# Project-SEA-Stack/HydroChrono

Measured on AMD Instinct MI355X. Metric: hydro-force evals/sec (all bodies), higher is better.
Workload: dtype f64

## Files before the change

hydrochrono_amd/csrc/hc_context.hpp:

```cpp
#pragma once
#include <hip/hip_runtime.h>

#include <chrono>
#include <cmath>
#include <deque>
#include <stdexcept>
#include <string>
#include <vector>

#include "../../include/hydrochrono_amd.h"
#include "hc_direct.hpp"
#include "hc_kernels.hpp"
#include "hc_plan.hpp"

namespace hc {

struct Error : std::runtime_error {
    int status;
    Error(int st, const std::string& what) : std::runtime_error(what), status(st) {}
};

#define HC_HIP(expr)                                                                                          \
    do {                                                                                                      \
        hipError_t _e = (expr);                                                                               \
// ... 126 lines not shown
    std::vector<std::vector<double>> tris;
    int items = 0, chunks = 0;
    std::vector<int> runs;
    DeviceBuffer<double> panel, tri, state, part, out;
    DeviceBuffer<int> chunk, off;
    PinnedBuffer<double> h_state, h_out;
    bool pts_dirty = true;
    DeviceBuffer<double> pt;
    DeviceBuffer<int> pbody;
    DeviceBuffer<int> pidx, tidx;
};

struct BodyHost {
    bool have_props = false, have_lin = false, have_ainf = false, have_rirf = false, have_rao = false, have_exirf = false;
    double disp_vol = 0.0, cg[3] = {0, 0, 0}, cb[3] = {0, 0, 0};
    double lin[36]  = {0};
    std::vector<double> ainf;
    std::vector<double> rao_w;
    std::vector<double> rao_mag;
    std::vector<double> rao_phase;
    std::vector<double> hd_dir;
    std::vector<double> hd_w;
    std::vector<double> hd_mag;
    std::vector<double> hd_phase;
    std::vector<double> exirf_t;
    std::vector<double> exirf_f;
};

struct StepTail {
    bool pending = false, rad = false, waves = false, block = false, direct = false, caller_waits = false;
    int m = 0, H = 0;
    hipStream_t stream = nullptr;
};

struct AheadPass {
    bool active = false;
    unsigned long long plan_serial = 0;
    int slices = 0, issued = 0;
    int per_slice = 0;
    bool reduced = false;
    bool concurrent = false;
    bool has_exc = false;
    int Hcap = 0;
    int head0 = 0, Hv = 0;
    double t_first = 0.0, t_last = 0.0;
    double rad_once = 0.0, exc_once = 0.0;
    BlockArgs args;
};

struct ExGroup {
    int first_body = 0, off = 0, L = 0;
    double tau_front = 0.0, tau_back = 0.0;
};

enum WaveKind { kWaveNone = 0, kWaveRegular = 1, kWaveIrregular = 2, kWaveSpectral = 3 };

enum EventKind { kEvConvPlain = 0, kEvPass = 1, kEvStep = 2, kEvScatter = 3, kEvConvExc = 4, kEvMiniPass = 5, kEvTail = 6 };
struct EventPair {
    hipEvent_t a = nullptr, b = nullptr;
    int kind = 0;
    double waves_share = 0.0;
};

}

struct hc_ctx {
    int N = 0, b0 = 0, b1 = 0, nloc = 0, D = 0, Dloc = 0, device = 0;
    hipStream_t stream = nullptr;
    hipStream_t stream_am = nullptr;
    hipEvent_t ev_fin = nullptr, ev_bg = nullptr;
    bool bg_pending = false;
    hipStream_t last_stream = nullptr;
    bool have_last_stream   = false;
    hc::DirectQueue* dq = nullptr;
    bool direct_ready   = false;
    std::string direct_why;
    std::string direct_how = "direct AQL dispatch";
    int path            = 0;
    hc::DirectKernel dk_finalize_slot;
    hc::DirectKernel dk_step_hot[2];
    bool step_hot = false;
    int step_halves = 1;
    bool slot_state = false;
    hc::DirectKernel dk_finalize, dk_scatter, dk_reduce, dk_block16, dk_block32, dk_block64, dk_mini16, dk_mini32, dk_narrow, dk_wide, dk_added_mass, dk_step, dk_near;
    hc::StepTail tail;
    int pending_step  = 0;
    double pending_t  = 0.0;
    int pending_am    = 0;
    bool lost         = false;
    int arm_mode = 1;
    bool arm_after_step = false, arm_after_am = false;
    std::chrono::steady_clock::time_point t_step_end{}, t_am_end{};
    bool have_t_step_end = false, have_t_am_end = false;
    int busy_caller_steps   = 0;
    std::string err;

    bool have_sim = false;
    double rho = 0, g = 0, depth = 0;
    double gsys[3] = {0.0, 0.0, -9.81};
    std::vector<hc::BodyHost> bodies;

    int S = 0;
    std::vector<double> tau, width;
    hc::DeviceBuffer<double> dK, dKproc, d_tau, d_width, d_stage;
    int ntiles = 0, Dpad = 0, ngp = 0, mt = 1, ngroups = 0;
    int conv_mode = 0;
    bool proc_ready = false;
    hc_tapered_direct_options taper{};
    std::string diagnostics_dir;
    bool finalized = false;

    std::deque<double> times;
    std::deque<double> retired;
    int head = -1, Hcap = 0, HcapT = 0;
    hc::DeviceBuffer<double> d_ring_t, d_ring_v, d_ring_vT;
    long long rewinds = 0;
    bool have_prev = false, have_prev_device = false;
    double prev_time = -1.0, prev_time_device = -1.0;

    hc::DeviceBuffer<double> d_lin, d_cg, d_cbmcg, d_vol, d_ainf, d_vec_w, d_vec_R;
    std::vector<double> ainf_host;

    int wave_kind = hc::kWaveNone;
    int wave_nb_arg = 0;
    double reg_amp = 0, reg_omega = 0, reg_wavenumber = 0;
    std::vector<double> reg_mag, reg_phase;
    hc::DeviceBuffer<double> d_reg_mag;
    hc_irregular_wave_params irr{};
    int eta_mode = 0;
    int L = 0, Lpad = 0, nf = 0, nt = 0;
    std::vector<double> ex_tau, ex_width, ex_vals;
    std::vector<hc::ExGroup> ex_groups;
    std::vector<int> ex_group_of;
    std::vector<double> spec_f, spec_S, spec_df, spec_phase, spec_k;
    std::vector<double> eta_t, eta;
    bool eta_record = false;
    std::vector<double> rec_t, rec_eta;
    double eta_h = 0.0;
    std::vector<int> rec_m;
    std::vector<double> rec_amp;
    double rec_mean = 0.0, rec_share = 0.0, rec_rms = 0.0;
    bool record_components() const { return wave_kind == hc::kWaveIrregular && eta_record && !rec_amp.empty(); }
    void drop_record_components() {
        rec_m.clear();
        rec_amp.clear();
        rec_mean = rec_share = rec_rms = 0.0;
    }
    hc::DeviceBuffer<double> d_kex, d_ex_tau, d_ex_width, d_eta_t, d_eta;
    hc::DeviceBuffer<double> d_spec_mag, d_spec_phase, d_spec_amp, d_spec_omega, d_spec_phi;
    unsigned long long wave_serial = 0;
    std::vector<double> wave_dir;

    hc::KinTableCopy kin;
    hc::DeviceBuffer<double> d_kin_io;

    hc::SideLane mor, nl;
    hc::Order2Part mor2, nl2;
    hc::MorisonData morison;
    hc::SurfaceData surface;

    hc::QtfTerm drift, sum;

    hipStream_t stream_wk2 = nullptr;
    hc::Wk2TableSet wk2;
    hc::DeviceBuffer<double> d_wk2_io;

    int chunk_gp = 0, nchunks_rad = 0, chunk_gp_ex = 0, nchunks_ex = 0, ngp_ex = 0;
// ... 98 lines not shown
```

hydrochrono_amd/csrc/hc_internal.hpp:

```cpp
#pragma once
#include <dlfcn.h>
#include <fcntl.h>
#include <unistd.h>
#include <xmmintrin.h>

#include <algorithm>
#include <chrono>
#include <cmath>
#include <cstdint>
#include <cstdio>
#include <cstdlib>
#include <cstring>
#include <fstream>
#include <limits>
#include <memory>
#include <string>
#include <vector>

#include "hc_context.hpp"
#include "hc_history.hpp"
#include "hc_host_math.hpp"

namespace hc {
void eta_synthesis_fft(const std::vector<double>& t, const std::vector<double>& amp, const std::vector<double>& omega,
// ... 61 lines not shown
#define HC_TUNE_INT(name, fallback) ::hc::detail::env_int(name, fallback)
#else
#define HC_TUNE_INT(name, fallback) (fallback)
#endif
void setup_panel_geometry(hc_ctx* c);
hc::Panel rad_panel(const hc_ctx* c);
void choose_conv_config(hc_ctx* c);
void choose_exc_config(hc_ctx* c);
void alloc_partials(hc_ctx* c);
int far_chunk_gp(const hc_ctx* c);
int far_chunks_per_slice(const hc_ctx* c);
int default_pass_slices(const hc_ctx* c);
int default_pass_ahead(const hc_ctx* c);
bool pass_ahead_size_ok(const hc_ctx* c);
bool pass_ahead_possible(const hc_ctx* c);
void reset_schedule_state(hc_ctx* c);
void ensure_processed(hc_ctx* c);
void check_device_flag(hc_ctx* c);
void stage_state(hc_ctx* c, const double* pos, const double* rpy, const double* linvel, const double* angvel);
std::string library_dir();
bool direct_selftest_rewrites(hc_ctx* c, hc::DirectQueue* q, int lane, bool* abandon);
void setup_direct(hc_ctx* c);

struct ExcitationGrid {
    std::vector<hc::ExGroup> groups;
    std::vector<int> group_of;
    std::vector<double> tau, width, vals;
    int L = 0;
    double tau_min = 0.0, tau_max = 0.0;
};
ExcitationGrid resample_excitation(hc_ctx* c, double dt);
void upload_excitation(hc_ctx* c, const ExcitationGrid& ex);
void commit_excitation(hc_ctx* c, ExcitationGrid& ex);
void drop_lookahead_excitation(hc_ctx* c);

struct RaoBracket {
    int k0, k1;
    double fr;
};
inline RaoBracket rao_bracket_clamped(double omega, double w_back, int nw) {
    const double dw = w_back / static_cast<double>(nw);
    double idx = omega / dw - 1;
    idx        = std::min(std::max(idx, 0.0), static_cast<double>(nw - 1));
    const int k0 = std::min(static_cast<int>(std::floor(idx)), nw - 2 >= 0 ? nw - 2 : 0);
    const int k1 = std::min(k0 + 1, nw - 1);
    return RaoBracket{k0, k1, idx - k0};
}
inline RaoBracket rao_bracket_regular(double omega, double w_back, int nw) {
    const double dw      = w_back / static_cast<double>(nw);
    const double idx_des = (omega / dw) - 1;
    const int k0         = static_cast<int>(std::floor(idx_des));
    return RaoBracket{k0, k0 + 1, idx_des - std::floor(idx_des)};
}
inline void rao_bracket_check(const RaoBracket& br, int nw) {
    if (br.k0 < 0 || br.k0 + 1 >= nw) throw Error(HC_ERR_OUT_OF_RANGE, "regular wave frequency outside the BEM frequency list");
}
void apply_wave_directions(hc_ctx* c, const std::vector<double>& theta, bool commit, bool force);

struct StepFlags {
    bool hs = true, rad = true, waves = true;
    bool scratch_out = false;
};
struct HostState {
    const double *pos, *rpy, *linvel, *angvel;
    double canary;
};
void enqueue_step(hc_ctx* c, double t, const double* d_state, double* d_user_out, hipStream_t stream, StepFlags f,
                  unsigned long long* host_tagged = nullptr, unsigned long long seq = 0, bool defer_tail = false, const HostState* host_state = nullptr);
void enqueue_tail(hc_ctx* c);

bool wave_window_ok(const hc_ctx* c, double t);
int live_samples(const hc_ctx* c, double t_query);
double* rows_P(hc_ctx* c, bool next);
double* rows_E(hc_ctx* c, bool next);

struct StepViews {
    hc::Panel kex;
    hc::EtaTable ex;
};
StepViews make_views(const hc_ctx* c);
struct PassSetup {
    hc::BlockArgs b;
    bool exc_block = false;
    double rad_once = 0.0, exc_once = 0.0, bytes_steps = 0.0;
};
PassSetup make_pass(hc_ctx* c, bool with_exc, bool next_block, int head_lags = 0);
void issue_pass_chunks(hc_ctx* c, const PassSetup& ps, int first, int last, bool with_items, hipStream_t stream, bool direct, int lane = 0);
struct TailRows {
    const double* tail[hc::kTailLevelsMax] = {nullptr, nullptr, nullptr};
    int j0[hc::kTailLevelsMax]             = {0, 0, 0};
};
void issue_pass_reduce(hc_ctx* c, const PassSetup& ps, double* P, double* E, hipStream_t stream, bool direct, int lane = 0, const TailRows* tail = nullptr);
void launch_pass(hc_ctx* c, hipStream_t stream, bool with_exc, bool direct = false, bool spec_goes_on = false);
void spec_drop(hc_ctx* c, bool k_changed);
void spec_build_khat(hc_ctx* c, hc_ctx::SpectralLevel& lev);
void launch_mini_pass(hc_ctx* c, int i0, hipStream_t stream, bool direct, int next_kw = 0, int lane = 0);
void ahead_drop(hc_ctx* c);
void ahead_issue_slice(hc_ctx* c, hipStream_t stream, bool direct);
void ahead_begin(hc_ctx* c, hipStream_t stream, bool with_exc, bool direct);
bool ahead_expected(const hc_ctx* c, unsigned long long ended_serial);
bool ahead_adoptable(const hc_ctx* c, unsigned long long ended_serial);
bool pass_lane_ready(hc_ctx* c);
void pass_lane_drain(hc_ctx* c);

}
}
```

hydrochrono_amd/csrc/hc_kernels.hip:

```cpp
#include "hc_kernels.hpp"

#include <algorithm>
#include <cstdint>
#include <cstdlib>

namespace hc {

static constexpr int kConvThreads = 256;
static constexpr int kWave        = 64;

typedef double dvec2 __attribute__((ext_vector_type(2)));
typedef double dvec2u __attribute__((ext_vector_type(2), aligned(8)));
typedef double dvec4 __attribute__((ext_vector_type(4)));

__host__ __device__ inline size_t panel_offset(int ngp, int row, int f) {
    const int rt = row >> 4, ri = row & 15, gp = f >> 3, j = (f >> 2) & 1, kk = f & 3;
    return ((static_cast<size_t>(rt) * ngp + gp) * 64 + (kk * 16 + ri)) * 2 + j;
}

__global__ void __launch_bounds__(256) relayout_rirf_kernel(const double* __restrict__ Kb, double* __restrict__ K, int ngp, int D, int S,
                                                             int row0, double scale) {
    const size_t F   = (size_t)S * D;
    const size_t gid = (size_t)blockIdx.x * blockDim.x + threadIdx.x;
    if (gid >= 6 * F) return;
// ... 768 lines not shown
        else block_rad_stream<MT, (NB > 1) ? 2 : R, NB, false>(a, chunk, grp, front, t_wo, t_wn, t_oo, t_on);
    }
    const int RG      = a.ngroups;
    const int n_items = a.nchunks_ex * NB * RG;
    if (n_items > 0) {
        __shared__ int s_item;
        for (;;) {
            __syncthreads();
            if (threadIdx.x == 0) s_item = atomicAdd(a.item_counter, 1);
            __syncthreads();
            const int it = s_item;
            if (it >= n_items) break;
            const int e = it / (NB * RG), rem = it - e * (NB * RG), tb = rem / RG, rg = rem - tb * RG;
            block_exc_work<MT>(a, rg, e, 16 * tb, front);
        }
    }
}

template <class KernelT>
static void allow_dynamic_lds(KernelT kernel, size_t smem, size_t& granted) {
    if (smem > 64 * 1024 && smem > granted) {
        (void)hipFuncSetAttribute(reinterpret_cast<const void*>(kernel), hipFuncAttributeMaxDynamicSharedMemorySize, (int)smem);
        granted = smem;
    }
}

template <int MT, int R>
static void launch_conv_block_mt(const BlockArgs& b, int nblocks, size_t smem, hipStream_t stream) {
    static size_t granted16 = 0, granted32 = 0;
    if (b.depth == 32) {
        allow_dynamic_lds(conv_block_kernel<MT, R + 1, 2>, smem, granted32);
        hipLaunchKernelGGL((conv_block_kernel<MT, R + 1, 2>), dim3(nblocks), dim3(kConvThreads), smem, stream, b);
    } else {
        allow_dynamic_lds(conv_block_kernel<MT, R, 1>, smem, granted16);
        hipLaunchKernelGGL((conv_block_kernel<MT, R, 1>), dim3(nblocks), dim3(kConvThreads), smem, stream, b);
    }
}

#ifdef HC_TUNING
static void launch_conv_block64(const BlockArgs& b, int nblocks, size_t smem, hipStream_t stream) {
    static size_t granted = 0;
    allow_dynamic_lds(conv_block_kernel<kBlock64MT, 4, 4, 1>, smem, granted);
    hipLaunchKernelGGL((conv_block_kernel<kBlock64MT, 4, 4, 1>), dim3(nblocks), dim3(kConvThreads), smem, stream, b);
}
#endif

BlockLaunch block_launch_config(const BlockArgs& a, int mt, BlockArgs* b) {
    BlockLaunch l;
    const int nlaunch = (a.chunk_last > 0 ? a.chunk_last : a.nchunks) - a.chunk_first;
    l.nblocks = ((nlaunch + 7) >> 3) * 8 * a.ngroups;
    *b        = a;
    b->lds_front_doubles = max(4 * kUWave, 4 * mt * 256);
    l.smem    = (size_t)b->lds_front_doubles * sizeof(double) + (size_t)max(1, a.max_steps_per_chunk) * b->depth * 24;
#ifdef HC_TUNING
    if (a.depth == 64) {
        l.MT  = kBlock64MT;
        l.NB  = 4;
        l.R   = 4;
        l.WPS = 1;
        return l;
    }
#endif
    l.MT  = (mt == 6 || mt == 4 || mt == 2) ? mt : 1;
    const int R16 = l.MT == 6 ? 3 : 4;
    l.NB  = a.depth == 32 ? 2 : 1;
    l.R   = a.depth == 32 ? R16 + 1 : R16;
    l.WPS = l.NB == 1 ? 2 : 1;
    return l;
}

void launch_conv_block(const BlockArgs& a, int mt, hipStream_t stream) {
    BlockArgs b;
    const BlockLaunch l = block_launch_config(a, mt, &b);
    const int nblocks   = l.nblocks;
    const size_t smem   = l.smem;
    if (nblocks <= 0) return;
#ifdef HC_TUNING
    if (b.depth == 64) { launch_conv_block64(b, nblocks, smem, stream); return; }
#endif
    if (mt == 6) launch_conv_block_mt<6, 3>(b, nblocks, smem, stream);
    else if (mt == 4) launch_conv_block_mt<4, 4>(b, nblocks, smem, stream);
    else if (mt == 2) launch_conv_block_mt<2, 4>(b, nblocks, smem, stream);
    else launch_conv_block_mt<1, 4>(b, nblocks, smem, stream);
}

__device__ __forceinline__ double lane16_sum(double v) {
#pragma unroll
    for (int off = 8; off >= 1; off >>= 1) v += __shfl_xor(v, off, 16);
    return v;
}

__global__ void __launch_bounds__(256) reduce_block_kernel(ReduceArgs a) {
    if (blockIdx.x == 0 && threadIdx.x == 0) *a.item_counter = 0;
    const double* __restrict__ partials = a.partials;
    const int sub = threadIdx.x & 15;
    const int n   = a.depth * a.Dpad;
    int out       = blockIdx.x * 16 + (threadIdx.x >> 4);
    const bool exc = out >= n;
    if (exc) out -= n;
    const int first = exc ? a.nchunks_rad : a.rad_first, count = exc ? a.nchunks_ex : a.nchunks_rad - a.rad_first;
    const int o     = out < n ? out : 0;
    double v = 0.0;
    if (a.narrow) {
        const int j = o / a.Dpad, row = o - j * a.Dpad;
        for (int c = sub; c < count; c += 8 * 16) {
            double w[8];
#pragma unroll
            for (int k = 0; k < 8; ++k) {
                const int cc = first + c + 16 * k;
                const int jj = (c + 16 * k) < count ? j - (int)a.jbase[cc] : -1;
                w[k]         = (jj >= 0 && jj < 16) ? partials[((size_t)cc * 16 + jj) * a.Dpad + row] : 0.0;
            }
#pragma unroll
            for (int k = 0; k < 8; ++k) v += w[k];
        }
    } else {
        for (int c = sub; c < count; c += 8 * 16) {
            double w[8];
#pragma unroll
            for (int k = 0; k < 8; ++k) w[k] = (c + 16 * k) < count ? partials[(size_t)(first + c + 16 * k) * n + o] : 0.0;
#pragma unroll
            for (int k = 0; k < 8; ++k) v += w[k];
        }
    }
    v = lane16_sum(v);
    if (out < n && sub == 0) {
        if (a.accumulate) {
            const int j = out / a.Dpad;
            if (!exc && j < a.j_cnt) a.P[out + (size_t)a.j_off * a.Dpad] += v;
        } else {
            if (!exc && a.tail) {
                const int j = out / a.Dpad, row = out % a.Dpad;
                v += a.tail[(size_t)(a.tail_j0 + j) * a.Dpad + row];
                if (a.tail_b) v += a.tail_b[(size_t)(a.tail_b_j0 + j) * a.Dpad + row];
                if (a.tail_c) v += a.tail_c[(size_t)(a.tail_c_j0 + j) * a.Dpad + row];
            }
            (exc ? a.E : a.P)[out] = v;
        }
    }
}

int reduce_block_grid(const ReduceArgs& r) {
    const int nblk = (r.depth * r.Dpad + 15) / 16;
    return r.nchunks_ex > 0 ? 2 * nblk : nblk;
}

void launch_reduce_block(const ReduceArgs& r, hipStream_t stream) {
    hipLaunchKernelGGL(reduce_block_kernel, dim3(reduce_block_grid(r)), dim3(256), 0, stream, r);
}

#ifdef HC_TUNING
struct StageClock {
    unsigned long long t[kStampStages] = {};
    template <int K>
    __device__ __forceinline__ void mark() {
#if defined(__HIP_DEVICE_COMPILE__)
        __builtin_amdgcn_sched_barrier(0);
        t[K] = __builtin_amdgcn_s_memrealtime();
        __builtin_amdgcn_sched_barrier(0);
#endif
    }
    __device__ __forceinline__ void store(unsigned long long* stamps) const {
        if (stamps && threadIdx.x == 0 && blockIdx.x < kStampWGs) {
#pragma unroll
            for (int k = 0; k < kStampStages; ++k) stamps[blockIdx.x * kStampStages + k] = t[k];
        }
// ... 1177 lines not shown
```

hydrochrono_amd/csrc/hc_kernels.hpp:

```cpp
#pragma once
#include <hip/hip_runtime.h>

#include <cstddef>

#include "hc_limits.hpp"
#include "hc_tail.hpp"

namespace hc {


struct Panel {
    const double* base;
    int ntiles;
    int ngp;
};
inline size_t panel_doubles(int ntiles, int ngp) { return static_cast<size_t>(ntiles) * ngp * 128; }

struct HistoryView {
    const double* state;
    int N, D;
    double t;
    const double* ring_t;
    const double* ring_v;
    const double* ring_vT;
// ... 177 lines not shown
    const double* v;
    const double* width;
    double* Y;
    int n_slices, gps_per_slice;
    int n_tgt[kScatterSamples];
    int tgt_off[kScatterSamples][kTargets];
    double tgt_coef[kScatterSamples][kTargets];
};

struct AddedMassArgs {
    const double* M;
    int rows, cols;
    const double *w, *R_in;
    double c;
    unsigned long long* tagged;
    unsigned long long seq;
    const double* canary_in;
    unsigned long long* canary_out;
};
static_assert(sizeof(AddedMassArgs) == 72, "kernarg layout of added_mass_mv_tagged_kernel");

struct ReduceArgs {
    const double* partials;
    int nchunks_rad, nchunks_ex, Dpad, depth;
    double *P, *E;
    int* item_counter;
    int accumulate, j_off, j_cnt;
    int rad_first;
    int narrow;
    int tail_j0;
    unsigned char jbase[kMiniChunks];
    const double* tail;
    const double* tail_b;
    const double* tail_c;
    int tail_b_j0, tail_c_j0;
};
static_assert(sizeof(ReduceArgs) == 104 + kMiniChunks && kMiniChunks % 8 == 0, "kernarg layout of reduce_block_kernel");

struct TaperArgs {
    Panel Kraw;
    double* Kproc;
    int Dloc, D, S;
    int effective_steps;
    int smoothing;
    int window;
    int tc_index, tc_end;
    double final_amplitude;
};

struct FinalizeLaunch {
    int grid = 0, threads = 256;
    size_t smem = 0;
};
struct NearLaunch {
    int grid = 0;
    size_t smem = 0;
};
int near_slices_for(int D);
NearLaunch near_launch_config(NearArgs& a);
struct WideLaunch {
    int grid = 0;
    size_t smem = 0;
};
WideLaunch wide_launch_config(WideStepArgs& a);
struct ScatterLaunch {
    int grid = 0;
    size_t smem = 0;
};
ScatterLaunch scatter_launch_config(ScatterArgs& a);
FinalizeLaunch finalize_launch_config(FinalizeArgs& a);
struct StepLaunch {
    int nblocks = 0;
    size_t smem = 0;
    int MT = 0;
    static constexpr int U = 2;
};
StepLaunch step_launch_config(const StepArgs& a, int mt);
struct BlockLaunch {
    int nblocks = 0;
    size_t smem = 0;
    int MT = 0, R = 0, NB = 0, WPS = 0;
};
BlockLaunch block_launch_config(const BlockArgs& a, int mt, BlockArgs* with_lds_layout);

void launch_relayout_rirf(const double* d_Kb_6xDxS, double* d_K, int ngp, int D, int S, int row0, double scale, hipStream_t stream);
void launch_relayout_rowmajor(const double* d_src, int rows, int cols, double* d_panel, int ngp, int row0, hipStream_t stream);
void launch_conv_step(const StepArgs& a, int mt, hipStream_t stream);
void launch_conv_block(const BlockArgs& a, int mt, hipStream_t stream);
void launch_reduce_block(const ReduceArgs& r, hipStream_t stream);
int reduce_block_grid(const ReduceArgs& r);
void launch_finalize(const FinalizeArgs& a, hipStream_t stream);
void launch_near_split(const NearArgs& a, hipStream_t stream);
void launch_wide_step(const WideStepArgs& a, hipStream_t stream);
void launch_scatter(const ScatterArgs& a, hipStream_t stream);
void launch_taper(const TaperArgs& a, hipStream_t stream);
void launch_eta_synthesis(const double* d_t, int nt, const double* d_amp, const double* d_omega, const double* d_phase, int nf,
                          double ramp_duration, double* d_eta, hipStream_t stream);
void launch_added_mass_mv(const double* d_M, int rows, int cols, const double* d_w, double c, double* d_R, hipStream_t stream);
void launch_added_mass_mv_tagged(const double* d_M, int rows, int cols, const double* d_w, const double* d_R_in, double c,
                                 unsigned long long* d_tagged, unsigned long long seq, const double* d_canary_in, unsigned long long* d_canary_out,
                                 hipStream_t stream);
void launch_unrelayout(const Panel& K, int Dloc, int D, int S, double* d_out, hipStream_t stream);
void launch_extract_series(const Panel& K, int row, int col, int D, int S, double* d_out, hipStream_t stream);
void launch_ring_transpose(const double* d_ring_v, int Hcap, int HcapT, int D, double* d_ring_vT, hipStream_t stream);
void launch_synth_rirf(double* d_K, int ntiles, int ngp, int Dloc, int D, int S, int row0, double dt, unsigned long long seed, double rho,
                       hipStream_t stream);

struct TailKhatArgs {
    Panel K;
    const double* width;
    const double* tw;
    double* Khat;
    int Dloc, D, S, NP;
};

struct TailFwdArgs {
    const double* ring_vT;
    int HcapT, Hcap, head;
    int D, S, NP;
    const double* tw;
    double* Xw;
};

struct TailGemvArgs {
    const double* Khat;
    const double* Xw;
    const double* Yin;
    double* Yout;
    int Dloc, ncols;
    int bin_lo, bin_hi;
    int col_lo, col_hi;
    int x_shift;
    int rows_per_wg;
};

struct TailInvArgs {
    const double* Y;
    const double* tw;
    double* tail;
    int Dloc, Dpad;
};
constexpr int kTailGemvRows = 32;
int tail_gemv_lds_bytes(const TailGemvArgs& g);
int tail_gemv_grid(const TailGemvArgs& g);
hipError_t launch_tail_khat(const TailKhatArgs& a, int N, hipStream_t s);
hipError_t launch_tail_fwd(const TailFwdArgs& a, int N, hipStream_t s);
void launch_tail_gemv(const TailGemvArgs& a, hipStream_t s);
hipError_t launch_tail_inv(const TailInvArgs& a, int N, hipStream_t s);

}
```

hydrochrono_amd/csrc/hc_pass.cpp:

```cpp
#include "hc_internal.hpp"

using namespace hc::detail;

namespace hc {
namespace detail {

StepViews make_views(const hc_ctx* c) {
    StepViews v{};
    const bool irregular = c->wave_kind == hc::kWaveIrregular;
    v.kex.base   = c->d_kex.p;
    v.kex.ntiles = c->ntiles;
    v.kex.ngp    = c->ngp_ex;
    v.ex.L        = c->L;
    v.ex.ex_tau   = c->d_ex_tau.p;
    v.ex.ex_width = c->d_ex_width.p;
    v.ex.eta_t    = c->d_eta_t.p;
    v.ex.eta      = c->d_eta.p;
    v.ex.nt       = c->nt;
    v.ex.eta_dt   = irregular ? (c->eta_record ? c->eta_h : c->irr.simulation_dt) : 1.0;
    v.ex.eta_t0   = (irregular && !c->eta_t.empty()) ? c->eta_t.front() : 0.0;
    return v;
}


PassSetup make_pass(hc_ctx* c, bool with_exc, bool next_block, int head_lags) {
    const bool head_only = head_lags > 0;
    auto& pl = c->plan;
    const int L = c->lookahead;
    const int H = static_cast<int>(c->times.size());
    const double hmin = pl.tgrid[1] - (c->tau.empty() ? 0.0 : c->tau.back());
    int Hv = H + 1;
    auto vtime = [&](int k) { return k == 0 ? pl.tgrid[1] : c->times[static_cast<size_t>(k - 1)]; };
    while (Hv > 1 && vtime(Hv - 2) < hmin) --Hv;

    hc::HistoryView hv{};
    hv.state   = c->d_zero_state.p;
    hv.N       = c->N;
    hv.D       = c->D;
    hv.t       = pl.tgrid[1];
    hv.ring_t  = c->d_ring_t.p;
    hv.ring_v  = c->d_ring_v.p;
    hv.ring_vT = c->d_ring_vT.p;
    hv.head    = (c->head + 1) % c->Hcap;
    hv.H       = Hv;
    hv.Hcap    = c->Hcap;
    hv.HcapT   = c->HcapT;
    hv.dt_hint = pl.dt;

    const StepViews vw = make_views(c);
    PassSetup ps;
    hc::BlockArgs& b = ps.b;
    b                     = hc::BlockArgs{};
    b.K                   = rad_panel(c);
    b.F                   = std::min(head_only ? head_lags : c->S, live_samples(c, pl.tgrid[L])) * c->D;
    b.depth               = L;
    b.chunk_gp            = next_block ? far_chunk_gp(c) : (head_only ? (head_lags < hc::kTailP ? c->chunk_gp_head128 : c->chunk_gp_head) : c->chunk_gp_block);
    b.nchunks             = std::max(1, ((b.F + 7) / 8 + b.chunk_gp - 1) / b.chunk_gp);
    b.max_steps_per_chunk = (b.chunk_gp * 8) / c->D + 2;
    b.hist                = hv;
    if (next_block) {
        const hc::FarPass fp = hc::far_pass_setup(pl, L, c->tau);
        for (int j = 0; j < L; ++j) {
            b.tpred[j]   = fp.tpred[j];
            b.s_cut[j]   = fp.s_cut[j];
            b.s_defer[j] = -1;
        }
    } else {
        for (int j = 0; j < L; ++j) {
            b.tpred[j]   = pl.tgrid[j + 1];
            b.s_cut[j]   = pl.s_cut[j];
            b.s_defer[j] = pl.s_defer[j];
        }
    }
    b.tau   = c->d_tau.p;
    b.width = c->d_width.p;
    static const bool exc_in_block = HC_TUNE_INT("HC_EXC_IN_BLOCK", 1) != 0;
    bool exc_block = exc_in_block && with_exc && c->wave_kind == hc::kWaveIrregular && c->nchunks_ex_block > 0;
    for (int j = 0; j < L && exc_block; ++j) exc_block = wave_window_ok(c, b.tpred[j]);
    ps.exc_block  = exc_block;
    b.Kex         = vw.kex;
    b.ex          = vw.ex;
    b.chunk_gp_ex = c->chunk_gp_ex_block;
    b.nchunks_ex  = exc_block ? c->nchunks_ex_block : 0;
    b.partials    = next_block ? c->d_partials_far.p : c->d_partials_block.p;
    b.Dpad        = c->Dpad;
    b.error_flag  = c->d_err.p;
    b.item_counter = c->d_err.p + 1;
    b.ngroups     = c->ntiles / (L == 64 ? hc::kBlock64MT : c->mt_block);
    double samples = 0.0;
    for (int j = 0; j < L; ++j) samples += std::max(0, b.F / c->D - b.s_cut[j]);
    const double rad_16 = 8.0 * samples * (static_cast<double>(c->Dloc) * c->D + c->D);
    const double exc_16 = exc_block ? 8.0 * L * (static_cast<double>(c->Dloc) * c->L + c->L) : 0.0;
    ps.bytes_steps = rad_16 + exc_16;
    ps.rad_once    = 8.0 * (static_cast<double>(c->Dloc) * b.F + b.F);
    ps.exc_once    = exc_block ? 8.0 * (static_cast<double>(c->Dloc) * c->L + c->L) : 0.0;
    if (HC_TUNE_INT("HC_DEBUG_PLAN", 0) != 0) {
        std::fprintf(stderr, "[hc] pass%s t0=%.6f dt=%.17g Hv=%d F/D=%d nchunks=%d exc=%d\n     s_cut:", next_block ? " (next block)" : "", pl.tgrid[0], pl.dt, Hv,
                     b.F / c->D, b.nchunks, (int)exc_block);
        for (int j = 0; j < L; ++j) std::fprintf(stderr, " %d", b.s_cut[j]);
        std::fprintf(stderr, "\n     s_defer:");
        for (int j = 0; j < L; ++j) std::fprintf(stderr, " %d", b.s_defer[j]);
        std::fprintf(stderr, "\n     scat:");
        for (int i = 1; i <= L; ++i) std::fprintf(stderr, " [%d,%d]", pl.scat_lo[i], pl.scat_hi[i]);
        std::fprintf(stderr, "\n");
    }
    return ps;
}

void issue_pass_chunks(hc_ctx* c, const PassSetup& ps, int first, int last, bool with_items, hipStream_t stream, bool direct, int lane) {
    hc::BlockArgs b = ps.b;
    b.chunk_first   = first;
    b.chunk_last    = last;
    if (!with_items) b.nchunks_ex = 0;
    const double share_rad = static_cast<double>(last - first) / std::max(1, ps.b.nchunks);
    const double rad_once = ps.rad_once * share_rad, exc_once = with_items ? ps.exc_once : 0.0;
    c->prof.block_kernel_bytes      = ps.bytes_steps * (rad_once + exc_once) / std::max(1.0, ps.rad_once + ps.exc_once);
    c->prof.block_kernel_bytes_once = rad_once + exc_once;
    const double exc_share = exc_once / std::max(1.0, rad_once + exc_once);
    const int L  = c->lookahead;
    const int mt = L == 64 ? hc::kBlock64MT : c->mt_block;
    if (direct) {
        hc::BlockArgs b2;
        const hc::BlockLaunch l = hc::block_launch_config(b, mt, &b2);
        if (l.nblocks <= 0) return;
        c->dq->dispatch(L == 64 ? c->dk_block64 : (L == 32 ? c->dk_block32 : c->dk_block16), static_cast<uint32_t>(l.nblocks), 256, static_cast<uint32_t>(l.smem), &b2, sizeof b2,
                        direct_tag(c, hc::kEvPass), exc_share, lane);
        c->prof.direct_dispatches += 1;
        if (lane == 2) c->prof.pass_lane_launches += 1;
        return;
    }
    hc::EventPair* ev = ev_begin(c, hc::kEvPass, stream, exc_share);
    hc::launch_conv_block(b, mt, stream);
    ev_end(ev, stream);
    c->prof.hip_launches += 1;
}

void issue_pass_reduce(hc_ctx* c, const PassSetup& ps, double* P, double* E, hipStream_t stream, bool direct, int lane, const TailRows* tail) {
    const hc::BlockArgs& b = ps.b;
    hc::ReduceArgs r{b.partials, b.nchunks, b.nchunks_ex, c->Dpad, c->lookahead, P, E, b.item_counter, 0, 0, 0, 0};
    if (tail) {
        r.tail      = tail->tail[0];
        r.tail_j0   = tail->j0[0];
        r.tail_b    = tail->tail[1];
        r.tail_b_j0 = tail->j0[1];
        r.tail_c    = tail->tail[2];
        r.tail_c_j0 = tail->j0[2];
    }
    if (direct) {
        c->dq->dispatch(c->dk_reduce, static_cast<uint32_t>(hc::reduce_block_grid(r)), 256, 0, &r, sizeof r, -1, 0.0, lane);
        c->prof.direct_dispatches += 1;
        return;
    }
    hc::launch_reduce_block(r, stream);
    c->prof.hip_launches += 1;
}

void spec_drop(hc_ctx* c, bool k_changed) {
    c->spec.active = false;
    c->spec.far_cur = c->spec.far_next = 0;
    if (k_changed)
        for (auto& f : c->spec_form) f.khat_ok = false;
}

namespace {

int spec_n_index(int N) { return N == 256 ? 0 : (N == 512 ? 1 : 2); }
int spec_form_index(const hc_ctx* c) { return c->radiation_tail == hc::kTailFormUniform ? 1 : 0; }

bool spec_eligible(const hc_ctx* c, bool direct) {
    const auto& pl = c->plan;
    if (c->radiation_tail != hc::kTailFormLevelled && c->radiation_tail != hc::kTailFormUniform) return false;
    hc::TailLevel lv[hc::kTailLevelsMax];
    const int nlev = hc::tail_levels(c->S, c->radiation_tail, lv);
    if (nlev < 1) return false;
    if (direct) {
        if (!c->dk_tail_gemv.ok()) return false;
        for (int l = 0; l < nlev; ++l)
            if (!c->dk_tail_fwd[spec_n_index(lv[l].N)].ok() || !c->dk_tail_inv[spec_n_index(lv[l].N)].ok()) return false;
    }
    if (c->conv_mode == 1 && !c->proc_ready) return false;
    if (c->pass_ahead == 1 || (c->pass_ahead == 2 && c->ahead_now && pass_ahead_size_ok(c))) return false;
    const int L = c->lookahead;
    const int NP = hc::tail_partitions(c->S);
    if ((L != 16 && L != 32) || c->D >= 1024 || NP < 1 || NP * c->D > hc::kTailMaxCols) return false;
    if (!pl.valid || pl.own_zero || pl.sub != 0) return false;
    const int head = hc::tail_head_lags(lv, nlev);
    for (int j = 0; j < L; ++j)
        if (pl.s_defer[j] >= 0 || pl.s_cut[j] >= head) return false;
    return hc::tail_grid_ok(c->times, c->tau, pl.dt, pl.tgrid[1]);
}

void spec_twiddles(hc_ctx* c, hc_ctx::SpectralLevel& lev) {
    const int N = lev.lv.N;
    if (lev.tw.n == static_cast<size_t>(2 * N)) return;
    std::vector<double> tw(2 * static_cast<size_t>(N));
    const double pi = 3.14159265358979323846;
    for (int k = 0; k < N; ++k) {
        const int q = (4 * k) / N, r = k - q * (N / 4);
        const double cr = std::cos(2.0 * pi * r / N), sr = std::sin(2.0 * pi * r / N);
        double co = cr, si = sr;
        if (q == 1) { co = -sr; si = cr; }
        if (q == 2) { co = -cr; si = -sr; }
        if (q == 3) { co = sr; si = -cr; }
// ... 450 lines not shown
```

hydrochrono_amd/csrc/hc_runtime.cpp:

```cpp
#include "hc_internal.hpp"

#include <sched.h>

#include <cctype>

#include <atomic>

using namespace hc::detail;

template <class T>
void hc::BarBuffer<T>::alloc(size_t count) {
    if (p) (void)hipFree(p);
    p       = nullptr;
    n       = 0;
    host_ok = false;
    if (count == 0) return;
    static const bool disabled = HC_TUNE_INT("HC_NO_BAR_STATE", 0) != 0;
    if (disabled) return;
    void* q = nullptr;
    if (hipExtMallocWithFlags(&q, count * sizeof(T), hipDeviceMallocFinegrained) != hipSuccess) {
        (void)hipGetLastError();
        return;
    }
    p = static_cast<T*>(q);
// ... 555 lines not shown
        }
        const unsigned long long bits = tag[0];
        double got;
        std::memcpy(&got, &bits, sizeof got);
        if (got != rv + cv * wv) {
            c->direct_why = "self-test of the direct dispatch: memory re-written through the PCIe BAR was read stale";
            (void)q->drain(2.0, lane);
            return false;
        }
    }
    if (!q->drain(2.0, lane)) {
        c->direct_why = "self-test of the direct dispatch timed out";
        *abandon      = true;
        return false;
    }
    return true;
}

#ifdef HC_TUNING
static const char* const kKernelObjectName = "/hc_kernels_tuning.co";
#else
static const char* const kKernelObjectName = "/hc_kernels.co";
#endif
__attribute__((constructor)) static void request_device_memory_queue_rings() {
    if (env_int("HC_QUEUE_DEV_MEM", 0) == 0) return;
    (void)setenv("HSA_ALLOCATE_QUEUE_DEV_MEM", "1", 0);
}

void setup_direct(hc_ctx* c) {
    c->direct_ready = false;
    if (env_int("HC_DIRECT", 1) == 0) { c->direct_why = "disabled by HC_DIRECT=0"; return; }
    if (!c->bar_state.host_ok || !c->bar_am.host_ok || !c->bar_selftest.host_ok) { c->direct_why = "the device's memory is not host-addressable"; return; }
    std::unique_ptr<hc::DirectQueue> q(new hc::DirectQueue);
    std::string why;
    if (!q->init(c->device, library_dir() + kKernelObjectName, &why)) { c->direct_why = why; return; }
    c->dk_finalize = q->find("finalize_kernelILi4ELb0EEEv");
    c->dk_finalize_slot = q->find("finalize_kernelILi4ELb1EEEv");
    c->dk_scatter  = q->find("scatter_kernelE");
    c->dk_near     = q->find("near_split_kernelE");
    c->dk_wide     = q->find("wide_step_kernelE");
    if (c->dk_wide.kernarg != sizeof(hc::WideStepArgs) || c->dk_wide.priv != 0) c->dk_wide = hc::DirectKernel{};
    if (c->dk_finalize_slot.kernarg != sizeof(hc::FinalizeArgs) || c->dk_finalize_slot.priv != 0) c->dk_finalize_slot = hc::DirectKernel{};
    c->slot_state = HC_TUNE_INT("HC_SLOT_STATE", 1) != 0 && c->dk_finalize_slot.ok() && c->N <= hc::kSlotStateMaxBodies;
    c->dk_step_hot[0] = q->find("step_hot_kernelILi1EEEv");
    c->dk_step_hot[1] = q->find("step_hot_kernelILi2EEEv");
    for (auto& k : c->dk_step_hot)
        if (k.kernarg != sizeof(hc::StepHotArgs) || k.priv != 0) k = hc::DirectKernel{};
    c->step_hot = c->slot_state && c->dk_step_hot[0].ok() && c->dk_step_hot[1].ok() && HC_TUNE_INT("HC_STEP_HOT", 1) != 0;
    c->step_halves = HC_TUNE_INT("HC_STEP_HALVES", 1) == 2 ? 2 : 1;
    c->dk_reduce   = q->find("reduce_block_kernelE");
    c->dk_tail_gemv = q->find("tail_gemvENS_12TailGemvArgsE");
    bool tail_ok    = c->dk_tail_gemv.kernarg == sizeof(hc::TailGemvArgs) && !c->dk_tail_gemv.priv;
    for (int i = 0; i < 3; ++i) {
        char frag[64];
        std::snprintf(frag, sizeof frag, "tail_fft_fwdILi%dEEEvNS_11TailFwdArgsE", 256 << i);
        c->dk_tail_fwd[i] = q->find(frag);
        std::snprintf(frag, sizeof frag, "tail_fft_invILi%dEEEvNS_11TailInvArgsE", 256 << i);
        c->dk_tail_inv[i] = q->find(frag);
        tail_ok = tail_ok && c->dk_tail_fwd[i].kernarg == sizeof(hc::TailFwdArgs) && c->dk_tail_inv[i].kernarg == sizeof(hc::TailInvArgs) && !c->dk_tail_fwd[i].priv &&
                  !c->dk_tail_inv[i].priv;
    }
    if (!tail_ok) {
        c->dk_tail_gemv = hc::DirectKernel{};
        for (int i = 0; i < 3; ++i) c->dk_tail_fwd[i] = c->dk_tail_inv[i] = hc::DirectKernel{};
    }
    c->dk_added_mass = q->find("added_mass_mv_tagged_kernelE");
    {
        hc::StepArgs a{};
        a.ngroups = 1;
        const hc::StepLaunch l = hc::step_launch_config(a, c->mt);
        char frag[64];
        std::snprintf(frag, sizeof frag, "conv_step_kernelILi%dELi%dEEEv", l.MT, hc::StepLaunch::U);
        c->dk_step = q->find(frag);
        if (c->dk_step.kernarg != sizeof(hc::StepArgs) || c->dk_step.priv != 0) c->dk_step = hc::DirectKernel{};
    }
    for (int depth : {16, 32}) {
        hc::BlockArgs a{}, b{};
        a.depth = depth;
        a.ngroups = 1;
        const hc::BlockLaunch l = hc::block_launch_config(a, c->mt_block, &b);
        char frag[96];
        std::snprintf(frag, sizeof frag, "conv_block_kernelILi%dELi%dELi%dELi%dEEEv", l.MT, l.R, l.NB, l.WPS);
        (depth == 16 ? c->dk_block16 : c->dk_block32) = q->find(frag);
        const hc::BlockLaunch lm = hc::block_launch_config(a, c->mt_mini, &b);
        std::snprintf(frag, sizeof frag, "conv_block_kernelILi%dELi%dELi%dELi%dEEEv", lm.MT, lm.R, lm.NB, lm.WPS);
        (depth == 16 ? c->dk_mini16 : c->dk_mini32) = q->find(frag);
        if (depth == 16) {
            const hc::BlockLaunch ln = hc::block_launch_config(a, c->mt_narrow, &b);
            std::snprintf(frag, sizeof frag, "conv_block_kernelILi%dELi%dELi%dELi%dEEEv", ln.MT, ln.R, ln.NB, ln.WPS);
            c->dk_narrow = q->find(frag);
        }
    }
#ifdef HC_TUNING
    {
        hc::BlockArgs a{}, b{};
        a.depth   = 64;
        a.ngroups = 1;
        const hc::BlockLaunch l = hc::block_launch_config(a, hc::kBlock64MT, &b);
        char frag[96];
        std::snprintf(frag, sizeof frag, "conv_block_kernelILi%dELi%dELi%dELi%dEEEv", l.MT, l.R, l.NB, l.WPS);
        c->dk_block64 = q->find(frag);
        if (c->dk_block64.kernarg != sizeof(hc::BlockArgs) || c->dk_block64.priv != 0) c->dk_block64 = hc::DirectKernel{};
    }
#endif
    if (!c->dk_narrow.ok() || c->dk_narrow.priv || c->dk_narrow.kernarg != sizeof(hc::BlockArgs)) {
        c->direct_why = "the narrow short-pass variant of the pass kernel is missing from hc_kernels.co";
        return;
    }
    if (!c->dk_mini16.ok() || !c->dk_mini32.ok() || c->dk_mini16.priv || c->dk_mini32.priv || c->dk_mini16.kernarg != sizeof(hc::BlockArgs) ||
        c->dk_mini32.kernarg != sizeof(hc::BlockArgs)) {
        c->direct_why = "the short-pass variant of the pass kernel is missing from hc_kernels.co";
        return;
    }
    if (!c->dk_finalize.ok() || !c->dk_scatter.ok() || !c->dk_reduce.ok() || !c->dk_block16.ok() || !c->dk_block32.ok() || !c->dk_near.ok()) {
        c->direct_why = "a kernel of this configuration is missing from hc_kernels.co";
        return;
    }
    if (c->dk_finalize.kernarg != sizeof(hc::FinalizeArgs) || c->dk_scatter.kernarg != sizeof(hc::ScatterArgs) ||
        c->dk_block16.kernarg != sizeof(hc::BlockArgs) || c->dk_block32.kernarg != sizeof(hc::BlockArgs) || c->dk_reduce.kernarg != sizeof(hc::ReduceArgs) ||
        c->dk_near.kernarg != sizeof(hc::NearArgs)) {
        c->direct_why = "hc_kernels.co was not built from the same sources as this library (argument block sizes differ)";
        return;
    }
    if (c->dk_finalize.priv || c->dk_scatter.priv || c->dk_reduce.priv || c->dk_block16.priv || c->dk_block32.priv || c->dk_near.priv) {
        c->direct_why = "a kernel needs scratch memory";
        return;
    }
    if (!c->dk_added_mass.ok() || c->dk_added_mass.kernarg != sizeof(hc::AddedMassArgs) || c->dk_added_mass.priv != 0) {
        c->direct_why = "added_mass_mv_tagged_kernel is missing from hc_kernels.co";
        return;
    }
    static_assert(hc::kSlotArgBytes == hc::DirectQueue::kSlotBytes && hc::kSlotStateDoubles * sizeof(double) == hc::DirectQueue::kExtraBytes &&
                      12 * hc::kSlotStateMaxBodies + 1 <= hc::kSlotStateDoubles && 6 * hc::kSlotStateMaxBodies <= 1024,
                  "the state behind the step kernel's arguments: hc_limits.hpp and hc_direct.hpp must agree");
    static_assert(sizeof(hc::NearArgs) <= hc::DirectQueue::kSlotBytes && sizeof(hc::WideStepArgs) <= hc::DirectQueue::kSlotBytes,
                  "an argument block does not fit a kernarg slot of the direct queue");
    static_assert(sizeof(hc::ScatterArgs) <= hc::DirectQueue::kSlotBytes && sizeof(hc::FinalizeArgs) <= hc::DirectQueue::kSlotBytes &&
                      sizeof(hc::BlockArgs) <= hc::DirectQueue::kSlotBytes && sizeof(hc::StepArgs) <= hc::DirectQueue::kSlotBytes,
                  "an argument block does not fit a kernarg slot of the direct queue");
    const double mark = 1.0;
    HC_HIP(hipMemcpy(c->d_P.p, &mark, sizeof mark, hipMemcpyHostToDevice));
    hc::ReduceArgs r{c->d_partials_block.p, 0, 0, c->Dpad, 1, c->d_P.p, c->d_E.p, c->d_err.p + 1, 0, 0, 0, 0};
    q->dispatch(c->dk_reduce, static_cast<uint32_t>((c->Dpad + 15) / 16), 256, 0, &r, sizeof r);
    if (!q->drain(2.0)) {
        c->direct_why = "self-test of the direct dispatch timed out";
        (void)q.release();
        return;
    }
    double back = -1.0;
    HC_HIP(hipMemcpy(&back, c->d_P.p, sizeof back, hipMemcpyDeviceToHost));
    if (back != 0.0) { c->direct_why = "self-test of the direct dispatch failed"; return; }
    {
        bool abandon = false;
        if (!direct_selftest_rewrites(c, q.get(), 0, &abandon)) {
            if (abandon) (void)q.release();
            return;
        }
    }
    c->dq           = q.release();
    c->direct_ready = true;
    c->direct_why.clear();
    {
        const int where = c->dq->ring_in_device_memory(0);
        c->direct_how   = where == 1 ? (c->dq->hdp_flush_available() ? "direct AQL dispatch (packet ring in device memory, HDP write-back in front of every doorbell)"
                                                                         : "direct AQL dispatch (packet ring in device memory, read-back in front of every doorbell: no HDP flush register)")
                          : where == 0 ? "direct AQL dispatch (packet ring in host memory; HC_QUEUE_DEV_MEM=1 moves the process's rings into device memory: "
// ... 9 lines not shown
```

Baseline: 84040.

## Add specialized head-only convolution block kernel for non-deferred passes

Adds a dedicated head_block_kernel that streams radiation kernel tiles and history-ring values with a register-pipelined issue/consume loop and MFMA f64 accumulation. It is used for head-only passes when the time grid is regular and no lags are deferred. It skips the general block kernel's tail/defer handling and per-wave slice bookkeeping, which is meant to cut instruction overhead on the hot per-step radiation convolution. The change adds another kernel variant with its own eligibility checks and direct-dispatch lookup, and it relies on those guards being correct.

```diff
diff --git a/hydrochrono_amd/csrc/hc_context.hpp b/hydrochrono_amd/csrc/hc_context.hpp
--- a/hydrochrono_amd/csrc/hc_context.hpp
+++ b/hydrochrono_amd/csrc/hc_context.hpp
@@ -232,7 +232,7 @@
     bool step_hot = false;
     int step_halves = 1;
     bool slot_state = false;
-    hc::DirectKernel dk_finalize, dk_scatter, dk_reduce, dk_block16, dk_block32, dk_block64, dk_mini16, dk_mini32, dk_narrow, dk_wide, dk_added_mass, dk_step, dk_near;
+    hc::DirectKernel dk_finalize, dk_scatter, dk_reduce, dk_block16, dk_block32, dk_block64, dk_head16, dk_head32, dk_mini16, dk_mini32, dk_narrow, dk_wide, dk_added_mass, dk_step, dk_near;
     hc::StepTail tail;
     int pending_step  = 0;
     double pending_t  = 0.0;
diff --git a/hydrochrono_amd/csrc/hc_internal.hpp b/hydrochrono_amd/csrc/hc_internal.hpp
--- a/hydrochrono_amd/csrc/hc_internal.hpp
+++ b/hydrochrono_amd/csrc/hc_internal.hpp
@@ -167,6 +167,7 @@
 struct PassSetup {
     hc::BlockArgs b;
     bool exc_block = false;
+    bool head_kernel = false;
     double rad_once = 0.0, exc_once = 0.0, bytes_steps = 0.0;
 };
 PassSetup make_pass(hc_ctx* c, bool with_exc, bool next_block, int head_lags = 0);
diff --git a/hydrochrono_amd/csrc/hc_kernels.hip b/hydrochrono_amd/csrc/hc_kernels.hip
--- a/hydrochrono_amd/csrc/hc_kernels.hip
+++ b/hydrochrono_amd/csrc/hc_kernels.hip
@@ -874,6 +874,206 @@
     else if (mt == 4) launch_conv_block_mt<4, 4>(b, nblocks, smem, stream);
     else if (mt == 2) launch_conv_block_mt<2, 4>(b, nblocks, smem, stream);
     else launch_conv_block_mt<1, 4>(b, nblocks, smem, stream);
+}
+
+template <int MT, int R, int NB>
+__device__ __forceinline__ void head_rad_stream(const BlockArgs& a, const int chunk, const int grp, double* red, double* wtab) {
+    constexpr int L = 16 * NB;
+    const int tid = threadIdx.x, lane = tid & 63;
+    const int wave = __builtin_amdgcn_readfirstlane(tid >> 6);
+    const int kk = lane >> 4, jstep = lane & 15;
+    const int D = a.hist.D;
+    const int gp0 = chunk * a.chunk_gp;
+    const int gp1 = min((a.F + 7) >> 3, gp0 + a.chunk_gp);
+    const int s0  = (gp0 * 8) / D;
+    const int ns  = (min(a.F, gp1 * 8) - 1) / D - s0 + 1;
+    const int s_live = a.F / D;
+    const int Hc = a.hist.HcapT, Hcap = a.hist.Hcap, head = a.hist.head, H = a.hist.H;
+
+    dvec4 acc[NB][MT];
+#pragma unroll
+    for (int tb = 0; tb < NB; ++tb)
+#pragma unroll
+        for (int m = 0; m < MT; ++m) acc[tb][m] = dvec4{0.0, 0.0, 0.0, 0.0};
+    const char* __restrict__ kb    = reinterpret_cast<const char*>(a.K.base) + ((size_t)(grp * MT) * a.K.ngp) * 1024;
+    const size_t tile_bytes        = (size_t)a.K.ngp * 1024;
+    const unsigned lane16          = (unsigned)lane * 16u;
+    const char* __restrict__ ringb = reinterpret_cast<const char*>(a.hist.ring_vT);
+    const unsigned col_bytes       = (unsigned)Hc * 8u;
+
+    const double w_mine = lane < ns ? a.width[s0 + lane] : 0.0;
+    int scut[NB];
+#pragma unroll
+    for (int tb = 0; tb < NB; ++tb) scut[tb] = a.s_cut[16 * tb + jstep];
+
+    dvec2 kv[R][MT];
+    double vk[R][2][NB];
+
+    auto live_k = [&](const int s, const int tb) {
+        const int k = s - (16 * tb + jstep);
+        return k >= 1 && k < H;
+    };
+    int gp_i = gp0 + wave;
+    int s_i = (gp_i * 8) / D, cb_i = gp_i * 8 - s_i * D;
+    unsigned cby = (unsigned)(cb_i + kk) * col_bytes;
+    unsigned boo[NB];
+    auto load_offsets = [&]() {
+#pragma unroll
+        for (int tb = 0; tb < NB; ++tb) {
+            int slot = head - (s_i - (16 * tb + jstep));
+            slot += slot < 0 ? Hcap : 0;
+            slot -= slot >= Hcap ? Hcap : 0;
+            boo[tb] = live_k(s_i, tb) ? (unsigned)slot * 8u : 0u;
+        }
+    };
+    load_offsets();
+    auto issue = [&](const int slot) {
+        const int gpc = min(gp_i, gp1 - 1);
+        const char* __restrict__ kg = kb + (size_t)gpc * 1024;
+#pragma unroll
+        for (int m = 0; m < MT; ++m) kv[slot][m] = __builtin_nontemporal_load(reinterpret_cast<const dvec2*>(kg + m * tile_bytes + lane16));
+#pragma unroll
+        for (int h = 0; h < 2; ++h)
+#pragma unroll
+            for (int tb = 0; tb < NB; ++tb) {
+                const unsigned cb = cby + (unsigned)(4 * h) * col_bytes;
+                vk[slot][h][tb]   = *reinterpret_cast<const double*>(ringb + (cb + boo[tb]));
+            }
+        gp_i += 4;
+        cb_i += 32;
+        cby += 32u * col_bytes;
+        if (cb_i >= D) {
+            do {
+                cb_i -= D;
+                cby -= (unsigned)D * col_bytes;
+                ++s_i;
+            } while (cb_i >= D);
+            load_offsets();
+        }
+    };
+
+    double* wt = wtab + wave * a.max_steps_per_chunk;
+    int gp_c = gp0 + wave;
+    int s_c = (gp_c * 8) / D, cb_c = gp_c * 8 - s_c * D;
+    double cw[NB];
+    auto load_weights = [&]() {
+        const int ks  = s_c - s0;
+        const bool in = ks >= 0 && ks < ns && s_c < s_live;
+        const double w = wt[in ? ks : 0];
+#pragma unroll
+        for (int tb = 0; tb < NB; ++tb) cw[tb] = (in && s_c >= scut[tb] && live_k(s_c, tb)) ? w : 0.0;
+    };
+    auto consume = [&](const int slot) {
+        if (gp_c < gp1) {
+            double u[2][NB];
+#pragma unroll
+            for (int h = 0; h < 2; ++h)
+#pragma unroll
+                for (int tb = 0; tb < NB; ++tb) u[h][tb] = cw[tb] * vk[slot][h][tb];
+#pragma unroll
+            for (int tb = 0; tb < NB; ++tb)
+#pragma unroll
+                for (int m = 0; m < MT; ++m) acc[tb][m] = __builtin_amdgcn_mfma_f64_16x16x4f64(kv[slot][m].x, u[0][tb], acc[tb][m], 0, 0, 0);
+#pragma unroll
+            for (int tb = 0; tb < NB; ++tb)
+#pragma unroll
+                for (int m = 0; m < MT; ++m) acc[tb][m] = __builtin_amdgcn_mfma_f64_16x16x4f64(kv[slot][m].y, u[1][tb], acc[tb][m], 0, 0, 0);
+        }
+        gp_c += 4;
+        cb_c += 32;
+        if (cb_c >= D) {
+            do {
+                cb_c -= D;
+                ++s_c;
+            } while (cb_c >= D);
+            load_weights();
+        }
+    };
+
+    const int nfrag = (gp1 - gp0 - wave + 3) / 4;
+#pragma unroll
+    for (int r = 0; r < R; ++r) issue(r);
+    if (lane < ns) wt[lane] = w_mine;
+    asm volatile("s_waitcnt lgkmcnt(0)" ::: "memory");
+    load_weights();
+    for (int i = 0; i < nfrag; i += R) {
+#pragma unroll
+        for (int r = 0; r < R; ++r) {
+            consume(r);
+            issue(r);
+        }
+    }
+
+#pragma unroll
+    for (int tb = 0; tb < NB; ++tb) {
+        __syncthreads();
+#pragma unroll
+        for (int m = 0; m < MT; ++m)
+#pragma unroll
+            for (int r = 0; r < 4; ++r) red[((size_t)wave * MT + m) * 256 + (kk + 4 * r) * 16 + jstep] = acc[tb][m][r];
+        __syncthreads();
+        for (int idx = tid; idx < MT * 256; idx += kConvThreads) {
+            const int m = idx >> 8, el = idx & 255, row = el >> 4, j = el & 15;
+            const double v = ((red[(0 * MT + m) * 256 + el] + red[(1 * MT + m) * 256 + el]) + red[(2 * MT + m) * 256 + el]) + red[(3 * MT + m) * 256 + el];
+            a.partials[((size_t)chunk * L + 16 * tb + j) * a.Dpad + (grp * MT + m) * 16 + row] = v;
+        }
+    }
+}
+
+template <int MT, int R, int NB>
+__global__ void __launch_bounds__(kConvThreads, 2) head_block_kernel(BlockArgs a) {
+    extern __shared__ __align__(16) unsigned char smem_raw[];
+    double* front = reinterpret_cast<double*>(smem_raw);
+    double* wtab  = front + a.lds_front_doubles;
+    const int RG    = a.ngroups;
+    const int n_rad = (((a.chunk_last > 0 ? a.chunk_last : a.nchunks) - a.chunk_first + 7) >> 3) * 8 * RG;
+    if ((int)blockIdx.x >= n_rad) {
+        const int it = (int)blockIdx.x - n_rad;
+        if (it >= a.nchunks_ex * NB * RG) return;
+        const int e = it / (NB * RG), rem = it - e * (NB * RG), tb = rem / RG, rg = rem - tb * RG;
+        block_exc_work<MT>(a, rg, e, 16 * tb, front);
+        return;
+    }
+    const int r     = (int)blockIdx.x % (8 * RG);
+    const int chunk = a.chunk_first + ((int)blockIdx.x / (8 * RG)) * 8 + (r & 7);
+    const int grp   = r >> 3;
+    if (chunk >= (a.chunk_last > 0 ? a.chunk_last : a.nchunks)) return;
+    head_rad_stream<MT, R, NB>(a, chunk, grp, front, wtab);
+}
+
+bool head_block_ok(const BlockArgs& a) {
+    return (a.depth == 16 || a.depth == 32) && (a.hist.D & 7) == 0 && (size_t)a.hist.D * a.hist.HcapT < ((size_t)1 << 28) && a.max_steps_per_chunk <= 64 &&
+           a.mini_kw == 0;
+}
+
+BlockLaunch head_launch_config(const BlockArgs& a, int mt, BlockArgs* b) {
+    BlockLaunch l;
+    const int nlaunch = (a.chunk_last > 0 ? a.chunk_last : a.nchunks) - a.chunk_first;
+    *b                = a;
+    l.MT  = (mt == 6 || mt == 4 || mt == 2) ? mt : 1;
+    l.NB  = a.depth == 32 ? 2 : 1;
+    l.R   = kHeadR;
+    l.WPS = 2;
+    l.nblocks = ((nlaunch + 7) >> 3) * 8 * a.ngroups + a.nchunks_ex * l.NB * a.ngroups;
+    b->lds_front_doubles = max(4 * kUWave, 4 * mt * 256);
+    l.smem = ((size_t)b->lds_front_doubles + 4 * (size_t)max(1, a.max_steps_per_chunk)) * sizeof(double);
+    return l;
+}
+
+template <int MT>
+static void launch_head_block_mt(const BlockArgs& b, int nblocks, size_t smem, hipStream_t stream) {
+    if (b.depth == 32) hipLaunchKernelGGL((head_block_kernel<MT, kHeadR, 2>), dim3(nblocks), dim3(kConvThreads), smem, stream, b);
+    else hipLaunchKernelGGL((head_block_kernel<MT, kHeadR, 1>), dim3(nblocks), dim3(kConvThreads), smem, stream, b);
+}
+
+void launch_head_block(const BlockArgs& a, int mt, hipStream_t stream) {
+    BlockArgs b;
+    const BlockLaunch l = head_launch_config(a, mt, &b);
+    if (l.nblocks <= 0) return;
+    if (mt == 6) launch_head_block_mt<6>(b, l.nblocks, l.smem, stream);
+    else if (mt == 4) launch_head_block_mt<4>(b, l.nblocks, l.smem, stream);
+    else if (mt == 2) launch_head_block_mt<2>(b, l.nblocks, l.smem, stream);
+    else launch_head_block_mt<1>(b, l.nblocks, l.smem, stream);
 }
 
 __device__ __forceinline__ double lane16_sum(double v) {
diff --git a/hydrochrono_amd/csrc/hc_kernels.hpp b/hydrochrono_amd/csrc/hc_kernels.hpp
--- a/hydrochrono_amd/csrc/hc_kernels.hpp
+++ b/hydrochrono_amd/csrc/hc_kernels.hpp
@@ -283,11 +283,15 @@
     int MT = 0, R = 0, NB = 0, WPS = 0;
 };
 BlockLaunch block_launch_config(const BlockArgs& a, int mt, BlockArgs* with_lds_layout);
+constexpr int kHeadR = 4;
+bool head_block_ok(const BlockArgs& a);
+BlockLaunch head_launch_config(const BlockArgs& a, int mt, BlockArgs* with_lds_layout);
 
 void launch_relayout_rirf(const double* d_Kb_6xDxS, double* d_K, int ngp, int D, int S, int row0, double scale, hipStream_t stream);
 void launch_relayout_rowmajor(const double* d_src, int rows, int cols, double* d_panel, int ngp, int row0, hipStream_t stream);
 void launch_conv_step(const StepArgs& a, int mt, hipStream_t stream);
 void launch_conv_block(const BlockArgs& a, int mt, hipStream_t stream);
+void launch_head_block(const BlockArgs& a, int mt, hipStream_t stream);
 void launch_reduce_block(const ReduceArgs& r, hipStream_t stream);
 int reduce_block_grid(const ReduceArgs& r);
 void launch_finalize(const FinalizeArgs& a, hipStream_t stream);
diff --git a/hydrochrono_amd/csrc/hc_pass.cpp b/hydrochrono_amd/csrc/hc_pass.cpp
--- a/hydrochrono_amd/csrc/hc_pass.cpp
+++ b/hydrochrono_amd/csrc/hc_pass.cpp
@@ -94,6 +94,11 @@
     ps.bytes_steps = rad_16 + exc_16;
     ps.rad_once    = 8.0 * (static_cast<double>(c->Dloc) * b.F + b.F);
     ps.exc_once    = exc_block ? 8.0 * (static_cast<double>(c->Dloc) * c->L + c->L) : 0.0;
+    if (head_only && !next_block && HC_TUNE_INT("HC_HEAD_KERNEL", 1) != 0 && hc::head_block_ok(b)) {
+        bool ok = hc::tail_grid_ok(c->times, c->tau, pl.dt, pl.tgrid[1]);
+        for (int j = 0; j < L && ok; ++j) ok = b.s_defer[j] < 0;
+        ps.head_kernel = ok;
+    }
     if (HC_TUNE_INT("HC_DEBUG_PLAN", 0) != 0) {
         std::fprintf(stderr, "[hc] pass%s t0=%.6f dt=%.17g Hv=%d F/D=%d nchunks=%d exc=%d\n     s_cut:", next_block ? " (next block)" : "", pl.tgrid[0], pl.dt, Hv,
                      b.F / c->D, b.nchunks, (int)exc_block);
@@ -119,6 +124,22 @@
     const double exc_share = exc_once / std::max(1.0, rad_once + exc_once);
     const int L  = c->lookahead;
     const int mt = L == 64 ? hc::kBlock64MT : c->mt_block;
+    if (ps.head_kernel && (!direct || (L == 32 ? c->dk_head32 : c->dk_head16).ok())) {
+        if (direct) {
+            hc::BlockArgs b2;
+            const hc::BlockLaunch l = hc::head_launch_config(b, mt, &b2);
+            if (l.nblocks <= 0) return;
+            c->dq->dispatch(L == 32 ? c->dk_head32 : c->dk_head16, static_cast<uint32_t>(l.nblocks), 256, static_cast<uint32_t>(l.smem), &b2, sizeof b2,
+                            direct_tag(c, hc::kEvPass), exc_share, lane);
+            c->prof.direct_dispatches += 1;
+            return;
+        }
+        hc::EventPair* ev = ev_begin(c, hc::kEvPass, stream, exc_share);
+        hc::launch_head_block(b, mt, stream);
+        ev_end(ev, stream);
+        c->prof.hip_launches += 1;
+        return;
+    }
     if (direct) {
         hc::BlockArgs b2;
         const hc::BlockLaunch l = hc::block_launch_config(b, mt, &b2);
diff --git a/hydrochrono_amd/csrc/hc_runtime.cpp b/hydrochrono_amd/csrc/hc_runtime.cpp
--- a/hydrochrono_amd/csrc/hc_runtime.cpp
+++ b/hydrochrono_amd/csrc/hc_runtime.cpp
@@ -661,6 +661,13 @@
         char frag[96];
         std::snprintf(frag, sizeof frag, "conv_block_kernelILi%dELi%dELi%dELi%dEEEv", l.MT, l.R, l.NB, l.WPS);
         (depth == 16 ? c->dk_block16 : c->dk_block32) = q->find(frag);
+        {
+            const hc::BlockLaunch lh = hc::head_launch_config(a, c->mt_block, &b);
+            std::snprintf(frag, sizeof frag, "head_block_kernelILi%dELi%dELi%dEEEv", lh.MT, lh.R, lh.NB);
+            hc::DirectKernel& dk = depth == 16 ? c->dk_head16 : c->dk_head32;
+            dk = q->find(frag);
+            if (dk.kernarg != sizeof(hc::BlockArgs) || dk.priv != 0) dk = hc::DirectKernel{};
+        }
         const hc::BlockLaunch lm = hc::block_launch_config(a, c->mt_mini, &b);
         std::snprintf(frag, sizeof frag, "conv_block_kernelILi%dELi%dELi%dELi%dEEEv", lm.MT, lm.R, lm.NB, lm.WPS);
         (depth == 16 ? c->dk_mini16 : c->dk_mini32) = q->find(frag);
```

Result: slower. 82930 (-1.3%).
